# matthewdm0816/BridgeQA

Hardware: AMD Instinct MI355X
Metric: train samples/s (40k-pt scene + 512^2 view, bs16) (higher is better)
Workload: dtype bf16

## Files before the change

bridgeqa_amd/_ext.py:

```python
import ctypes
import os

import torch

from . import _cabi

_LIB_PATH = os.environ.get("BQHIP_LIB") or os.path.join(os.path.dirname(os.path.abspath(__file__)), "lib", "libbqhip.so")

if not os.path.exists(_LIB_PATH):
    raise ImportError(
        "bridgeqa_amd: %s is missing -- build it with `python -m bridgeqa_amd.build` "
        "(hipcc --offload-arch=gfx950). There is no CPU fallback." % _LIB_PATH)

_lib = ctypes.CDLL(_LIB_PATH)
_D = _cabi.DEFINES
_cabi.bind(_lib, ("bq_abi_version", "bq_last_error"))
ABI_VERSION = _D["BQHIP_ABI_VERSION"]
if _lib.bq_abi_version() != ABI_VERSION:
    raise ImportError("bridgeqa_amd: libbqhip.so ABI %d != %d (stale library: python -m bridgeqa_amd.build --force)"
                      % (_lib.bq_abi_version(), ABI_VERSION))
_cabi.bind(_lib)
_cabi.bind(_lib, _cabi.ADDITIVE_PROTOS)

DET_ROUTES = {
# ... 1092 lines not shown

GEMM_P_XC, GEMM_Q_XC, GEMM_OUT_F32, GEMM_BACKGROUND = (_D["BQ_GEMM_" + n] for n in ("P_XC", "Q_XC", "OUT_F32", "BACKGROUND"))
EPI_NONE, EPI_BIAS, EPI_BIAS_GELU, EPI_DGELU, EPI_BIAS_CE, EPI_ADD = (
    _D["BQ_GEMM_EPI_" + n] for n in ("NONE", "BIAS", "BIAS_GELU", "DGELU", "BIAS_CE", "ADD"))
GEMM_DET = _D["BQ_GEMM_DET"]
_GemmDesc = _cabi.STRUCTS["bq_gemm_desc"]
GEMM_TILE_ROWS = 1024


def _mat(t, name):
    if not t.is_cuda:
        raise RuntimeError("%s: CPU not supported (bridgeqa_amd has no CPU path)" % name)
    if t.dim() != 2 or t.stride(1) != 1:
        raise RuntimeError("%s must be a 2-D tensor with a contiguous last dimension" % name)
    return t


def _mat_rows(t, name):
    if not t.is_cuda:
        raise RuntimeError("%s: CPU not supported (bridgeqa_amd has no CPU path)" % name)
    if t.dim() == 2:
        if t.stride(1) != 1:
            raise RuntimeError("%s must have a contiguous last dimension" % name)
        return (t.shape[0], t.shape[1]), t.stride(0), 0, 0
    if t.dim() != 3 or t.stride(2) != 1:
        raise RuntimeError("%s must be (rows, cols) or a (batch, rows, cols) view with a contiguous last dimension" % name)
    B, R, C = t.shape
    ld, bs = t.stride(1), t.stride(0)
    if B == 1 or bs == R * ld:
        return (B * R, C), ld, 0, 0
    if bs < R * ld or bs % 8 or R > 65535:
        raise RuntimeError("%s: unsupported batched-row view (stride %s, shape %s)" % (name, t.stride(), tuple(t.shape)))
    return (B * R, C), ld, R, bs


TILE256_MIN_K = [2304]


def pick_tile(Ni, Nj, q_xc, mid_ok=False):
    if Nj >= GEMM_TILE_ROWS and Ni >= 256:
        return 128 if mid_ok else 256
    if q_xc or Nj > 512:
        return 64
    return 32


def gemm_grouped(problems, flags, epilogue=EPI_NONE, tile=None, fixed_order=False):
    if _det() or fixed_order:
        return _gemm_grouped_det(problems, flags, epilogue, tile)
    return _gemm_grouped_launch(problems, flags, epilogue, tile)


def _gemm_grouped_launch(problems, flags, epilogue, tile):
    pxc, qxc, f32 = bool(flags & GEMM_P_XC), bool(flags & GEMM_Q_XC), bool(flags & GEMM_OUT_F32)
    n = len(problems)
    arr = (_GemmDesc * n)()
    t_auto = 32
    any_map = False
    for k, pr in enumerate(problems):
        P, Q, out = _mat(pr["P"], "P"), pr["Q"], pr["out"]
        qshape, ldq, q_rpb, q_bs = _mat_rows(Q, "Q")
        oshape, ldo, o_rpb, o_bs = _mat_rows(out, "out")
        any_map = any_map or bool(q_rpb or o_rpb)
        if P.dtype != torch.bfloat16 or Q.dtype != torch.bfloat16:
            raise RuntimeError("gemm: operands must be bf16")
        if out.dtype != (torch.float32 if f32 else torch.bfloat16):
            raise RuntimeError("gemm: out must be %s" % ("float32" if f32 else "bfloat16"))
        Ni, Kc = (P.shape[1], P.shape[0]) if pxc else (P.shape[0], P.shape[1])
        Nj, Kq = (qshape[1], qshape[0]) if qxc else (qshape[0], qshape[1])
        Ni = int(pr.get("Ni", Ni))
        if (Kq != Kc and "Kc" not in pr) or tuple(oshape) != (Nj, Ni):
            raise RuntimeError("gemm: shape mismatch P%s Q%s out%s" % (tuple(P.shape), tuple(Q.shape), tuple(out.shape)))
        d = arr[k]
        d.P, d.Q, d.out = P.data_ptr(), Q.data_ptr(), out.data_ptr()
        bias, out2, aux, colsum = pr.get("bias"), pr.get("out2"), pr.get("aux"), pr.get("colsum")
        if bias is not None and (bias.dtype not in (torch.float32, torch.bfloat16) or bias.numel() != Ni
                                 or not bias.is_contiguous()):
            raise RuntimeError("gemm: bias must be a contiguous fp32 or bf16 (Ni,) tensor")
        d.bias_bf16 = int(bias is not None and bias.dtype == torch.bfloat16)
        n_cs = Nj if (pxc and qxc and f32) else Ni
        if epilogue != EPI_BIAS_CE and colsum is not None and (colsum.dtype != torch.float32 or colsum.numel() != n_cs
                                                               or not colsum.is_contiguous()):
            raise RuntimeError("gemm: colsum must be a contiguous fp32 (%d,) tensor" % n_cs)
        for t, nm in ((out2, "out2"), (aux, "aux")):
            if epilogue != EPI_BIAS_CE and t is not None and (t.dtype != torch.bfloat16 or t.shape != out.shape
                                                              or t.stride() != out.stride()):
                raise RuntimeError("gemm: %s must be bf16 and laid out like out" % nm)
        d.bias, d.out2, d.aux, d.colsum = _p(bias), _p(out2), _p(aux), _p(colsum)
        d.ldp, d.ldq, d.ldo = P.stride(0), ldq, ldo
        d.q_rpb, d.q_bstride, d.o_rpb, d.o_bstride = q_rpb, q_bs, o_rpb, o_bs
        d.accum = int(bool(pr.get("accum", False)))
        d.Ni, d.Nj, d.Kc = Ni, Nj, Kc
        d.p_bytes, d.q_bytes, d.ksplit = int(pr.get("p_bytes", 0)), int(pr.get("q_bytes", 0)), int(pr.get("ksplit", 1))
        if "Kc" in pr:
            d.Kc = int(pr["Kc"])
        mid_ok = (not qxc and not f32 and d.Kc >= 128 and colsum is None
                  and epilogue in (EPI_NONE, EPI_BIAS, EPI_BIAS_GELU, EPI_DGELU, EPI_ADD))
        all_mid_ok = mid_ok if k == 0 else (all_mid_ok and mid_ok)
        t_auto = max(t_auto, pick_tile(Ni, Nj, qxc, True))
    if t_auto == 128 and not all_mid_ok:
        t_auto = 256
    if (t_auto == 128 and TILE256_MIN_K[0] and not pxc and epilogue in (EPI_NONE, EPI_BIAS)
            and all(int(arr[k].Kc) >= TILE256_MIN_K[0] for k in range(n))):
        t_auto = 256
    if t_auto == 256 and any_map and tile is None and not (pxc and qxc and f32):
        t_auto = 64
    dev = problems[0]["out"].device
    if (tile or t_auto) != 128:
        flags &= ~GEMM_BACKGROUND
    with torch.cuda.device(dev):
        if (tile or t_auto) == 128 and n == 1 and (STREAMK[0] or STREAMK256[0]):
            _streamk_workspace(dev)
        _check(_lib.bq_gemm_bf16(arr, n, int(flags), int(epilogue), int(tile or t_auto), _stream()), "gemm_bf16")


def _gemm_grouped_det(problems, flags, epilogue, tile):
    if _det() and (STREAMK[0] or STREAMK256[0]):
        raise RuntimeError("gemm: stream-K is on (streamk_enable / streamk256_enable) while the deterministic mode is on")
    f32 = bool(flags & GEMM_OUT_F32)
    probs, folds, sums = [], [], []
    for pr in problems:
        ks = int(pr.get("ksplit", 1))
        if epilogue != EPI_BIAS_CE and ks > 1:
            out = pr["out"]
            if not f32 or pr.get("colsum") is not None or pr.get("accum") or out.dim() != 2 or out.stride(1) != 1:
                raise RuntimeError("gemm: a cut contraction in the deterministic mode needs fp32 plain-row out, no colsum or accum")
            slab = torch.empty(ks, out.shape[0], out.stride(0), dtype=torch.float32, device=out.device)
            folds.append((slab, out, ks))
            pr = dict(pr, out=slab[0, :, :out.shape[1]])
        elif not f32 and epilogue != EPI_BIAS_CE and pr.get("colsum") is not None:
            sums.append((pr["out"], pr["colsum"]))
            pr = dict(pr, colsum=None)
        probs.append(pr)
    _gemm_grouped_launch(probs, flags | GEMM_DET, epilogue, tile)
    for slab, out, ks in folds:
        R, C = out.shape
        with torch.cuda.device(out.device):
            _check(_det_entry("gemm_splitk_fold")(_p(slab), _p(out), None, ks, R, C, out.stride(0), _stream()),
                   "gemm_splitk_fold_det")
    if sums:
        _colsum_grouped_into([o.reshape(-1, o.shape[-1]) if o.dim() == 3 else o for o, _ in sums], [c for _, c in sums],
                             "gemm_epilogue_colsum")


STREAMK = [False]
STREAMK256 = [os.environ.get("BQ_GEMM_STREAMK256", "0") == "1"]
_SK_WS = {}


def _streamk_apply():
    on = STREAMK[0] or STREAMK256[0]
    _lib.bq_gemm_streamk_mode((1 if STREAMK[0] else 0) | (2 if STREAMK256[0] else 0))
    for (d, sp), (ws, st) in _SK_WS.items():
        with torch.cuda.device(d):
            _check(_lib.bq_gemm_set_workspace(_p(ws) if on else None, ws.numel() if on else 0, sp), "gemm_set_workspace")


def streamk_enable(flag):
    STREAMK[0] = bool(flag)
    _streamk_apply()


def streamk256_enable(flag):
    STREAMK256[0] = bool(flag)
    _streamk_apply()


_streamk_apply()


# ... 465 lines not shown
```

bridgeqa_amd/csrc/gemm.hip:

```cpp
#include "gemm_common.h"

namespace bq {

typedef unsigned u32x4_sk __attribute__((ext_vector_type(4)));

template <bool P_XC, bool Q_XC, int EPI, bool OUT_F32, bool SK = false>
__global__ __launch_bounds__(512) void gemm256_kernel(const GemmArgs args) {
  static_assert(!SK || (!P_XC && !Q_XC && !OUT_F32 && (EPI == EPI_NONE || EPI == EPI_BIAS)), "stream-K: K-contiguous operands, bf16 out");
  __shared__ __attribute__((aligned(16))) unsigned char smem[131072];
  __shared__ unsigned s_skflag;
  constexpr bool GTAB = !OUT_F32 && (EPI == EPI_BIAS_GELU || EPI == EPI_DGELU);
  __shared__ float s_gtab[GTAB ? GELU_TAB_N : 1];
  const int tid = threadIdx.x;
  const int lane = tid & 63;
  const int wave = __builtin_amdgcn_readfirstlane(tid >> 6);
  const int wr = wave >> 2, wc = wave & 3;

  const int nwg = args.total_tiles;
  auto xcd_order = [](int b, int n) {
    const int q = n >> 3, r = n & 7, x = b & 7;
    return (x < r ? x * (q + 1) : r * (q + 1) + (x - r) * q) + (b >> 3);
  };
  const int G = (int)gridDim.x;
  const int nkt_full = SK ? (args.p[0].Kc + 63) >> 6 : 1;
  const int U = SK ? nwg * nkt_full : 0;
  auto bound = [&](int x) {
    int b = (int)((long)x * U / G);
    const int r = b % nkt_full;
    return r == 1 ? b - 1 : (r == nkt_full - 1 ? b + 1 : b);
  };
  const int slot = SK ? xcd_order((int)blockIdx.x, G) : 0;
  int su = SK ? bound(slot) : 0;
  const int sue = SK ? bound(slot + 1) : 0;
  if (SK && su >= sue) return;
  for (;;) {
  int t, kb = 0, kseg = 0;
  if (SK) {
    t = su / nkt_full;
    kb = su - t * nkt_full;
    kseg = min(nkt_full - kb, sue - su);
  } else {
    t = xcd_order((int)blockIdx.x, nwg);
  }
  int pi = 0;
  for (int k = 1; k < args.n; ++k)
    if (t >= args.p[k].tile0) pi = k;
  const GemmProblem &pr = args.p[pi];
  const int tl = t - pr.tile0;
  const int tiles_j = (pr.Nj + 255) >> 8;
  const int bj = tiles_j - 1 - tl / pr.tiles_i(), bi = tl % pr.tiles_i();
  const int i0 = bi * 256, j0 = bj * 256;
  const int Ni = pr.Ni, Nj = pr.Nj, Kc = pr.Kc;
  const int ldp = pr.ldp, ldq = pr.ldq;
  const int nkt = SK ? kseg : (Kc + 63) >> 6;

  const auto rsP = __builtin_amdgcn_make_buffer_rsrc((void *)pr.P, 0, pr.p_bytes, 0x00020000);
  const auto rsQ = __builtin_amdgcn_make_buffer_rsrc((void *)pr.Q, 0, pr.q_bytes, 0x00020000);
  const int ur = wave * 8 + (lane >> 3);
  const int cp = lane & 7;
  unsigned voff[8];
#pragma unroll
  for (int u = 0; u < 4; ++u) {
    const int g = u & 1, half = u >> 1;
    if (!P_XC) {
      const int c = cp ^ (ur & 7);
      voff[u] = (unsigned)(((i0 + g * 128 + half * 64 + ur) * ldp + c * 8) * 2);
    } else {
      const int c = cp ^ (xg(ur) << 1);
      voff[u] = (unsigned)((ur * ldp + i0 + g * 128 + half * 64 + c * 8) * 2);
    }
  }
#pragma unroll
  for (int u = 0; u < 4; ++u) {
    const int h = u & 1, half = u >> 1;
    if (!Q_XC) {
      const int c = cp ^ (ur & 7);
      voff[4 + u] = (unsigned)(((j0 + h * 128 + (ur >> 5) * 64 + half * 32 + (ur & 31)) * ldq + c * 8) * 2);
    } else {
      const int c = cp ^ (xg(ur) << 1);
      voff[4 + u] = (unsigned)((ur * ldq + j0 + h * 128 + (c >> 2) * 64 + half * 32 + (c & 3) * 8) * 2);
    }
  }
  const unsigned p_step = P_XC ? (unsigned)(64 * ldp * 2) : 128u;
  const unsigned q_step = Q_XC ? (unsigned)(64 * ldq * 2) : 128u;
  if (SK) {
#pragma unroll
    for (int u = 0; u < 4; ++u) { voff[u] += (unsigned)kb * p_step; voff[4 + u] += (unsigned)kb * q_step; }
  }
  const unsigned lds_w = (unsigned)(wave * 1024);
  const int q_rpb = Q_XC ? (int)pr.q_rpb() : 0;
  const unsigned q_gap = (unsigned)((pr.q_bstride - q_rpb * ldq) * 2);
  int q_rl[2] = {ur, ur};

  auto stage_pair = [&](int u, int kt) {
    const bool live = kt < nkt;
    const unsigned base = (unsigned)((kt & 1) * 65536 + u * 8192) + lds_w;
#pragma unroll
    for (int d = 0; d < 2; ++d) {
      const unsigned vo = live ? voff[u + d] : 0x80000000u;
      __builtin_amdgcn_raw_ptr_buffer_load_lds(u < 4 ? rsP : rsQ, (lds_void_t *)(smem + base + d * 8192), 16, vo, 0, 0, 0);
      voff[u + d] += (u < 4) ? p_step : q_step;
    }
    if (Q_XC && u >= 4 && q_rpb != 0) {
      int &rl = q_rl[(u - 4) >> 1];
      rl += 64;
      const bool wrap = rl >= q_rpb;
      rl -= wrap ? q_rpb : 0;
      voff[u] += wrap ? q_gap : 0u;
      voff[u + 1] += wrap ? q_gap : 0u;
    }
  };

  const int row16 = lane & 15, q4 = lane >> 4;
  const int kc_base = row16 * 128 + ((q4 ^ (row16 & 7)) << 4);
  int xc_base[4];
  {
    const int q = (lane & 15) >> 2, p = lane & 3, g = (q >> 1) | ((q4 & 1) << 1);
#pragma unroll
    for (int s = 0; s < 4; ++s) xc_base[s] = (8 * q4 + q) * 128 + ((s ^ g) << 5) + 8 * p;
  }
  const int uA0 = wr * 8192, uA1 = (2 + wr) * 8192, uB0 = (4 + (wc >> 1)) * 8192, uB1 = (6 + (wc >> 1)) * 8192;
  const int bsub = (wc & 1) * 2;

  const int iw = i0 + wr * 128, jw = j0 + wc * 64;
  const bool vA0 = iw < Ni, vA1 = iw + 64 < Ni, vB0 = jw < Nj, vB1 = jw + 32 < Nj;

  f32x4 acc[8][4];
#pragma unroll
  for (int a = 0; a < 8; ++a)
#pragma unroll
    for (int b = 0; b < 4; ++b) acc[a][b] = f32x4{0.f, 0.f, 0.f, 0.f};

  constexpr bool QSUM = P_XC && Q_XC && OUT_F32;
  const bool do_qsum = QSUM && pr.colsum != nullptr && bi == 0 && wr == 0;
  f32x4 qs[4];
  bf16x8 ones;
#pragma unroll
  for (int b = 0; b < 4; ++b) qs[b] = f32x4{0.f, 0.f, 0.f, 0.f};
#pragma unroll
  for (int e = 0; e < 8; ++e) ones[e] = (__bf16)1.0f;
#define BQ_MFMA_QSUM(FB, BO)                                                                          \
  if (QSUM && do_qsum) {                                                                              \
    _Pragma("unroll") for (int kk = 0; kk < 2; ++kk) _Pragma("unroll") for (int b = 0; b < 2; ++b)    \
        qs[BO + b] = __builtin_amdgcn_mfma_f32_16x16x32_bf16(ones, FB[b][kk], qs[BO + b], 0, 0, 0);   \
  }

  stage_pair(0, 0); stage_pair(4, 0); stage_pair(6, 0); stage_pair(2, 0); stage_pair(0, 1); stage_pair(4, 1); stage_pair(6, 1);
  if (GTAB) gelu_tab_fill<EPI == EPI_DGELU>(s_gtab, tid, 512);
  asm volatile("s_waitcnt vmcnt(8)" ::: "memory");
  BQ_BARRIER();
  if (wr == 1) BQ_BARRIER();

  bf16x8 fa[4][2], fb0[2][2], fb1[2][2];
  const unsigned smem_lds = lds_addr_of(smem);
#define BQ_MFMA_Q(AO, FB, BO)                                                                         \
  _Pragma("unroll") for (int kk = 0; kk < 2; ++kk) _Pragma("unroll") for (int a = 0; a < 4; ++a)      \
      _Pragma("unroll") for (int b = 0; b < 2; ++b) acc[AO + a][BO + b] =                             \
          __builtin_amdgcn_mfma_f32_16x16x32_bf16(fa[a][kk], FB[b][kk], acc[AO + a][BO + b], 0, 0, 0);
#define BQ_PHASE_SYNC_A()                                   \
  asm volatile("s_waitcnt vmcnt(8)" ::: "memory");          \
  asm volatile("s_waitcnt lgkmcnt(0)" ::: "memory");        \
  BQ_BARRIER();                                             \
  __builtin_amdgcn_sched_barrier(0);                        \
  __builtin_amdgcn_s_setprio(1);
#define BQ_PHASE_SYNC_B()                                   \
  __builtin_amdgcn_s_setprio(0);                            \
  BQ_BARRIER();

  for (int kt = 0; kt < nkt; ++kt) {
    const unsigned buf = smem_lds + (unsigned)((kt & 1) * 65536);
    if (vA0) {
#pragma unroll
      for (int a = 0; a < 4; ++a)
#pragma unroll
        for (int kk = 0; kk < 2; ++kk) fa[a][kk] = read_frag_asm<P_XC>(buf + uA0, a, kk, kc_base, xc_base);
    }
    if (vB0) {
#pragma unroll
      for (int b = 0; b < 2; ++b)
#pragma unroll
        for (int kk = 0; kk < 2; ++kk) fb0[b][kk] = read_frag_asm<Q_XC>(buf + uB0, bsub + b, kk, kc_base, xc_base);
    }
    if (vB1) {
#pragma unroll
      for (int b = 0; b < 2; ++b)
#pragma unroll
        for (int kk = 0; kk < 2; ++kk) fb1[b][kk] = read_frag_asm<Q_XC>(buf + uB1, bsub + b, kk, kc_base, xc_base);
    }
    stage_pair(2, kt + 1);
    BQ_PHASE_SYNC_A();
    if (vA0 && vB0) { BQ_MFMA_Q(0, fb0, 0) }
    if (vB0) { BQ_MFMA_QSUM(fb0, 0) }
    if (vA0 && vB1) { BQ_MFMA_Q(0, fb1, 2) }
    if (vB1) { BQ_MFMA_QSUM(fb1, 2) }
    BQ_PHASE_SYNC_B();
    if (vA1) {
#pragma unroll
      for (int a = 0; a < 4; ++a)
#pragma unroll
        for (int kk = 0; kk < 2; ++kk) fa[a][kk] = read_frag_asm<P_XC>(buf + uA1, a, kk, kc_base, xc_base);
    }
    stage_pair(0, kt + 2); stage_pair(4, kt + 2); stage_pair(6, kt + 2);
    BQ_PHASE_SYNC_A();
    if (vA1 && vB1) { BQ_MFMA_Q(4, fb1, 2) }
    if (vA1 && vB0) { BQ_MFMA_Q(4, fb0, 0) }
    BQ_PHASE_SYNC_B();
  }
  if (wr == 0) BQ_BARRIER();
  asm volatile("s_waitcnt vmcnt(0)" ::: "memory");
  BQ_BARRIER();

  if (SK && kseg != nkt_full) {
    unsigned *tick = (unsigned *)args.sk_ws + 2 * t;
    const int t0 = t * nkt_full, t1 = t0 + nkt_full;
    int s_lo = slot, s_hi = slot;
    while (s_lo > 0 && bound(s_lo) > t0) --s_lo;
    while (s_hi + 1 < G && bound(s_hi + 1) < t1) ++s_hi;
    const int n_part = s_hi - s_lo + 1;
    if (tid == 0) s_skflag = __hip_atomic_fetch_add(tick, 1u, __ATOMIC_RELAXED, __HIP_MEMORY_SCOPE_AGENT);
    __syncthreads();
    const unsigned arrived = (unsigned)__builtin_amdgcn_readfirstlane((int)s_skflag);
    constexpr unsigned SLAB256 = 256u * 256u * 4u;
    const auto rsW = __builtin_amdgcn_make_buffer_rsrc((char *)args.sk_ws + SK_TICKET_BYTES, 0, 0x7fffffffu, 0x00020000);
    auto slab_off = [&](int sl) { return (unsigned)(2 * sl + (bound(sl) >= t0 ? 0 : 1)) * SLAB256; };
    if (arrived != (unsigned)(n_part - 1)) {
      const unsigned base = slab_off(slot) + (unsigned)(tid * 16);
#pragma unroll
      for (int a = 0; a < 8; ++a)
#pragma unroll
        for (int b = 0; b < 4; ++b)
          __builtin_amdgcn_raw_buffer_store_b128(__builtin_bit_cast(u32x4_sk, acc[a][b]), rsW, base + (unsigned)((a * 4 + b) * 8192), 0, 16);
      asm volatile("s_waitcnt vmcnt(0)" ::: "memory");
      __syncthreads();
      if (tid == 0) __hip_atomic_fetch_add(tick + 1, 1u, __ATOMIC_RELAXED, __HIP_MEMORY_SCOPE_AGENT);
      su += kseg;
      if (su >= sue) return;
      continue;
    }
    if (tid == 0) {
      for (int spin = 0; spin < (1 << 22) && __hip_atomic_load(tick + 1, __ATOMIC_RELAXED, __HIP_MEMORY_SCOPE_AGENT) != (unsigned)(n_part - 1); ++spin)
        __builtin_amdgcn_s_sleep(4);
      __hip_atomic_store(tick, 0u, __ATOMIC_RELAXED, __HIP_MEMORY_SCOPE_AGENT);
      __hip_atomic_store(tick + 1, 0u, __ATOMIC_RELAXED, __HIP_MEMORY_SCOPE_AGENT);
    }
    __syncthreads();
    for (int sl = s_lo; sl <= s_hi; ++sl) {
      if (sl == slot) continue;
      const unsigned base = slab_off(sl) + (unsigned)(tid * 16);
#pragma unroll
      for (int a0 = 0; a0 < 8; a0 += 2) {
        u32x4_sk part[8];
#pragma unroll
        for (int e = 0; e < 8; ++e) part[e] = __builtin_amdgcn_raw_buffer_load_b128(rsW, base + (unsigned)((a0 * 4 + e) * 8192), 0, 16);
        asm volatile("s_waitcnt vmcnt(0)" ::: "memory");
        __builtin_amdgcn_sched_barrier(0);
#pragma unroll
        for (int e = 0; e < 8; ++e) acc[a0 + (e >> 2)][e & 3] += __builtin_bit_cast(f32x4, part[e]);
      }
    }
  }

  const int ldo = pr.ldo;
  if (OUT_F32) {
    float *out = reinterpret_cast<float *>(pr.out);
    if (QSUM && do_qsum && q4 == 0) {
#pragma unroll
      for (int b = 0; b < 4; ++b) {
        const int j = jw + b * 16 + row16;
        if (j < Nj) pr.colsum[j] = qs[b][0];
      }
    }
#pragma unroll
    for (int b = 0; b < 4; ++b) {
      const int j = jw + b * 16 + row16;
#pragma unroll
      for (int a = 0; a < 8; ++a) {
        const int i = iw + a * 16 + q4 * 4;
        if (j < Nj && i < Ni) {
          float4 *dst = reinterpret_cast<float4 *>(out + (long)j * ldo + i);
          const f32x4 v = acc[a][b];
          *dst = make_float4(v[0], v[1], v[2], v[3]);
        }
      }
    }
    return;
  }
  if (EPI == EPI_BIAS_CE) {
    const int n_valid = pr.ksplit();
    float *part = reinterpret_cast<float *>(pr.out2) + (long)(bi * 2 + wr) * Nj * 3;
    const int *tgt = reinterpret_cast<const int *>(pr.aux);
#pragma unroll
    for (int b = 0; b < 4; ++b) {
      const int j = jw + b * 16 + row16;
      const int t = j < Nj ? tgt[j] : -100;
      float m = -INFINITY, sz = 0.f;
#pragma unroll
      for (int a = 0; a < 8; ++a) {
        const int i = iw + a * 16 + q4 * 4;
        float bv[4] = {0.f, 0.f, 0.f, 0.f};
        if (pr.bias != nullptr && i < Ni) load_bias4(pr, i, bv);
#pragma unroll
        for (int r = 0; r < 4; ++r) {
          const float z = acc[a][b][r] + bv[r];
          if (i + r < n_valid) {
            m = fmaxf(m, z);
            sz += z;
            if (i + r == t) pr.colsum[j] = z;
          }
        }
      }
      float se = 0.f;
#pragma unroll
      for (int a = 0; a < 8; ++a) {
        const int i = iw + a * 16 + q4 * 4;
        float bv[4] = {0.f, 0.f, 0.f, 0.f};
        if (pr.bias != nullptr && i < Ni) load_bias4(pr, i, bv);
#pragma unroll
        for (int r = 0; r < 4; ++r)
          if (i + r < n_valid) se += __builtin_amdgcn_exp2f((acc[a][b][r] + bv[r] - m) * 1.4426950408889634f);
      }
#pragma unroll
      for (int sh = 16; sh <= 32; sh <<= 1) {
        const float mo = __shfl_xor(m, sh), so = __shfl_xor(se, sh), zo = __shfl_xor(sz, sh);
        const float mn = fmaxf(m, mo);
        const float fa = m == -INFINITY ? 0.f : __builtin_amdgcn_exp2f((m - mn) * 1.4426950408889634f);
        const float fb = mo == -INFINITY ? 0.f : __builtin_amdgcn_exp2f((mo - mn) * 1.4426950408889634f);
        se = se * fa + so * fb;
        m = mn;
        sz += zo;
      }
      if (q4 == 0 && j < Nj) {
        part[(long)j * 3 + 0] = m;
        part[(long)j * 3 + 1] = se;
        part[(long)j * 3 + 2] = sz;
      }
    }
  }
  unsigned char *ep = smem + wave * 16384;
  __bf16 *outb = reinterpret_cast<__bf16 *>(pr.out);
  const int npass = (EPI == EPI_BIAS_GELU) ? 2 : 1;
  const bool want_colsum = EPI != EPI_BIAS_CE && pr.colsum != nullptr;
#pragma unroll 1
  for (int pass = 0; pass < npass; ++pass) {
    if (EPI == EPI_DGELU || EPI == EPI_ADD) {
      float cs[8][4];
#pragma unroll
      for (int a = 0; a < 8; ++a)
#pragma unroll
        for (int r = 0; r < 4; ++r) cs[a][r] = 0.f;
      const auto rsX = __builtin_amdgcn_make_buffer_rsrc((void *)pr.aux, 0, (int)((long)Nj * ldo * 2), 0x00020000);
      uint2 yy[2][8];
      auto fetch = [&](int b, uint2(&dst)[8]) {
        const unsigned off = (unsigned)(((jw + b * 16 + row16) * ldo + iw + q4 * 4) * 2);
// ... 749 lines not shown
        }
        if (long_k) {
          hipLaunchKernelGGL((gemm64_kernel<32, P_XC, Q_XC, EPI, OUT_F32, 2>), dim3(ga.total_tiles), dim3(256), 0, st, ga);
          return 0;
        }
      }
      hipLaunchKernelGGL((gemm64_kernel<32, P_XC, Q_XC, EPI, OUT_F32>), dim3(ga.total_tiles), dim3(256), 0, st, ga);
    } else {
      return -1;
    }
  }
  return 0;
}

template <bool P_XC, bool Q_XC, int EPI>
static int launch_det_variant(const GemmArgs &ga, int tile, hipStream_t st) {
  if (tile == 64) {
    hipLaunchKernelGGL((gemm64_kernel_det<64, P_XC, Q_XC, EPI>), dim3(ga.total_tiles), dim3(256), 0, st, ga);
    return 0;
  }
  if constexpr (!Q_XC) {
    hipLaunchKernelGGL((gemm64_kernel_det<32, P_XC, Q_XC, EPI>), dim3(ga.total_tiles), dim3(256), 0, st, ga);
    return 0;
  }
  return -1;
}

static int launch_gemm(const GemmArgs &ga, int flags, int epi, int tile, hipStream_t st) {
  const bool pxc = flags & BQ_GEMM_P_XC, qxc = flags & BQ_GEMM_Q_XC, f32 = flags & BQ_GEMM_OUT_F32;
  if ((flags & BQ_GEMM_DET) && f32 && tile != 256 && tile != 128) {
    if (!pxc && !qxc && epi == EPI_NONE) return launch_det_variant<false, false, EPI_NONE>(ga, tile, st);
    if (!pxc && !qxc && epi == EPI_BIAS) return launch_det_variant<false, false, EPI_BIAS>(ga, tile, st);
    if (pxc && !qxc && epi == EPI_NONE) return launch_det_variant<true, false, EPI_NONE>(ga, tile, st);
    if (pxc && qxc && epi == EPI_NONE) return launch_det_variant<true, true, EPI_NONE>(ga, tile, st);
    return -1;
  }
  constexpr int long_k_tiles = 12;
  bool long_k = long_k_tiles > 0 && tile != 256 && ga.total_tiles <= 2048;
  for (int k = 0; k < ga.n; ++k) long_k = long_k && ga.p[k].Kc >= 64 * long_k_tiles;
  if (tile == 128 && (gemm_sk_mode() & 2) && !(flags & (BQ_GEMM_BACKGROUND | BQ_GEMM_DET)) && ga.n == 1 && !pxc && !qxc && !f32 &&
      (epi == EPI_NONE || epi == EPI_BIAS) && ga.p[0].colsum == nullptr && ga.p[0].q_rpb() == 0 && ga.p[0].o_rpb() == 0) {
    const GemmProblem &p0 = ga.p[0];
    const int cus = device_cus();
    const int nkt = (p0.Kc + 63) >> 6, tiles = ((p0.Ni + 255) / 256) * ((p0.Nj + 255) / 256);
    const long units = (long)tiles * nkt;
    const int rounds = (tiles + cus - 1) / cus;
    long ws_bytes = 0;
    void *ws = gemm_sk_workspace(st, &ws_bytes);
    if (ws != nullptr && nkt >= 24 && tiles >= cus / 2 && units / cus >= 16 && (long)rounds * nkt * cus >= units * 115 / 100 &&
        8L * tiles <= SK_TICKET_BYTES && ws_bytes >= SK_TICKET_BYTES + 2L * cus * 256 * 256 * 4) {
      GemmArgs g2 = ga;
      g2.sk_ws = ws;
      g2.total_tiles = tiles;
      g2.p[0].tile0 = 0;
      g2.p[0].tiles_ks = (p0.Ni + 255) / 256;
      if (epi == EPI_NONE) hipLaunchKernelGGL((gemm256_kernel<false, false, EPI_NONE, false, true>), dim3(cus), dim3(512), 0, st, g2);
      else hipLaunchKernelGGL((gemm256_kernel<false, false, EPI_BIAS, false, true>), dim3(cus), dim3(512), 0, st, g2);
      return 0;
    }
  }
  if (tile == 128)
    return launch_gemm_mid(ga, pxc, qxc, f32, epi, (flags & BQ_GEMM_BACKGROUND) != 0, st);
  if (!pxc && !qxc && !f32) {
    if (epi == EPI_NONE) return launch_variant<false, false, EPI_NONE, false>(ga, tile, st, long_k);
    if (epi == EPI_BIAS) return launch_variant<false, false, EPI_BIAS, false>(ga, tile, st, long_k);
    if (epi == EPI_BIAS_GELU) return launch_variant<false, false, EPI_BIAS_GELU, false>(ga, tile, st, long_k);
    if (epi == EPI_DGELU) return launch_variant<false, false, EPI_DGELU, false>(ga, tile, st, long_k);
    if (epi == EPI_ADD) return launch_variant<false, false, EPI_ADD, false>(ga, tile, st, long_k);
    if (epi == EPI_BIAS_CE && tile == 256) {
      hipLaunchKernelGGL((gemm256_kernel<false, false, EPI_BIAS_CE, false>), dim3(ga.total_tiles), dim3(512), 0, st, ga);
      return 0;
    }
  } else if (!pxc && !qxc && f32) {
    if (epi == EPI_NONE && tile != 256) return launch_variant<false, false, EPI_NONE, true>(ga, tile, st);
    if (epi == EPI_BIAS && tile != 256) return launch_variant<false, false, EPI_BIAS, true>(ga, tile, st);
  } else if (pxc && !qxc && f32) {
    if (epi == EPI_NONE && tile != 256) return launch_variant<true, false, EPI_NONE, true>(ga, tile, st);
  } else if (pxc && !qxc && !f32) {
    if (epi == EPI_NONE) return launch_variant<true, false, EPI_NONE, false>(ga, tile, st, long_k);
    if (epi == EPI_DGELU) return launch_variant<true, false, EPI_DGELU, false>(ga, tile, st, long_k);
    if (epi == EPI_ADD) return launch_variant<true, false, EPI_ADD, false>(ga, tile, st, long_k);
  } else if (pxc && qxc && f32) {
    if (epi == EPI_NONE) return launch_variant<true, true, EPI_NONE, true>(ga, tile, st);
  }
  return -1;
}

}

extern "C" int bq_gemm_max_problems(void) { return bq::GEMM_MAX_PROBLEMS; }

extern "C" int bq_gemm_bf16(const bq_gemm_desc *d, int n, int flags, int epilogue, int tile, void *stream) {
  using namespace bq;
  BQ_REQUIRE(d != nullptr && n >= 1, BQ_EINVAL, "bq_gemm_bf16: no problems");
  BQ_REQUIRE(tile == 256 || tile == 128 || tile == 64 || tile == 32, BQ_EINVAL,
             "bq_gemm_bf16: tile must be 256, 128 (= 256 x 128), 64 or 32 (got %d)", tile);
  const bool pxc = flags & BQ_GEMM_P_XC, qxc = flags & BQ_GEMM_Q_XC, f32 = flags & BQ_GEMM_OUT_F32;
  BQ_REQUIRE(!(flags & BQ_GEMM_BACKGROUND) || tile == 128, BQ_EINVAL, "bq_gemm_bf16: BQ_GEMM_BACKGROUND needs tile 128");
  const bool det = flags & BQ_GEMM_DET;
  BQ_REQUIRE(!det || tile != 128 || gemm_sk_mode() == 0, BQ_EINVAL,
             "bq_gemm_bf16: BQ_GEMM_DET with a stream-K mode on (bq_gemm_streamk_mode)");
  hipStream_t st = (hipStream_t)stream;
  int done = 0;
  while (done < n) {
    GemmArgs ga;
    ga.n = 0;
    ga.total_tiles = 0;
    while (done < n && ga.n < GEMM_MAX_PROBLEMS) {
      const bq_gemm_desc &s = d[done];
      BQ_REQUIRE(s.P && s.Q && s.out, BQ_EINVAL, "bq_gemm_bf16: null operand (problem %d)", done);
      BQ_REQUIRE(s.Ni > 0 && s.Nj > 0 && s.Kc > 0, BQ_EINVAL, "bq_gemm_bf16: empty problem %d", done);
      BQ_REQUIRE(s.ldp % 8 == 0 && s.ldq % 8 == 0, BQ_EINVAL, "bq_gemm_bf16: operand leading dimensions must be multiples of 8 elements");
      BQ_REQUIRE(s.Ni % 8 == 0 && s.ldo % (f32 ? 4 : 8) == 0, BQ_EINVAL, "bq_gemm_bf16: Ni and ldo must be multiples of 8 (Ni = %d, ldo = %d)", s.Ni, s.ldo);
      BQ_REQUIRE(!qxc || s.Nj % 8 == 0, BQ_EINVAL, "bq_gemm_bf16: a contraction-major Q needs Nj %% 8 == 0 (Nj = %d)", s.Nj);
      BQ_REQUIRE((pxc && qxc) || s.Kc % 64 == 0, BQ_EINVAL,
                 "bq_gemm_bf16: a K-contiguous operand needs Kc %% 64 == 0 (Kc = %d; zero-pad the other operand and pass "
                 "p_bytes / q_bytes when the rows are shorter)", s.Kc);
      BQ_REQUIRE(((uintptr_t)s.P % 16 == 0) && ((uintptr_t)s.Q % 16 == 0) && ((uintptr_t)s.out % 16 == 0), BQ_EINVAL,
                 "bq_gemm_bf16: operands must be 16-byte aligned");
      BQ_REQUIRE(epilogue != EPI_BIAS_GELU || s.out2, BQ_EINVAL, "bq_gemm_bf16: BIAS_GELU needs out2");
      BQ_REQUIRE(epilogue != EPI_DGELU || s.aux, BQ_EINVAL, "bq_gemm_bf16: DGELU needs aux");
      BQ_REQUIRE(epilogue != EPI_ADD || s.aux, BQ_EINVAL, "bq_gemm_bf16: ADD needs aux");
      BQ_REQUIRE((epilogue != EPI_ADD && epilogue != EPI_DGELU && tile != 128) || ((long)s.Nj + 256) * s.ldo * (f32 ? 4 : 2) < 0x7FFFFFFFL,
                 BQ_EINVAL, "bq_gemm_bf16: out / aux larger than 2 GB (problem %d)", done);
      const long pb = pxc ? ((long)(s.Kc - 1) * s.ldp + s.Ni) * 2 : ((long)(s.Ni - 1) * s.ldp + s.Kc) * 2;
      long qb = qxc ? ((long)(s.Kc - 1) * s.ldq + s.Nj) * 2 : ((long)(s.Nj - 1) * s.ldq + s.Kc) * 2;
      const int tj = tile == 256 ? 256 : tile, ti = (tile == 256 || tile == 128) ? 256 : 64;
      BQ_REQUIRE(s.q_rpb >= 0 && s.o_rpb >= 0 && s.q_rpb <= 65535 && s.o_rpb <= 65535, BQ_EINVAL,
                 "bq_gemm_bf16: q_rpb / o_rpb must be in 0..65535 (problem %d)", done);
      long q_span = 0, o_span = 0;
      if (s.q_rpb > 0) {
        const long rows = qxc ? s.Kc : s.Nj, cols = qxc ? s.Nj : s.Kc;
        BQ_REQUIRE(rows % s.q_rpb == 0 && s.q_bstride % 8 == 0 && (long)s.q_bstride >= (long)s.q_rpb * s.ldq, BQ_EINVAL,
                   "bq_gemm_bf16: q map: rows %ld must be whole batches of q_rpb = %d rows, q_bstride %% 8 == 0 and >= q_rpb * ldq",
                   rows, s.q_rpb);
        BQ_REQUIRE(tile != 256 || (qxc && s.q_rpb >= 64), BQ_EINVAL,
                   "bq_gemm_bf16: tile 256 maps only the contraction rows of a contraction-major Q, q_rpb >= 64");
        BQ_REQUIRE(tile != 128 || !qxc, BQ_EINVAL, "bq_gemm_bf16: tile 128 has no map on a contraction-major Q");
        q_span = (rows / s.q_rpb - 1) * (long)s.q_bstride + (long)(s.q_rpb - 1) * s.ldq + cols;
        qb = q_span * 2;
      }
      if (s.o_rpb > 0) {
        BQ_REQUIRE(s.Nj % s.o_rpb == 0 && s.o_bstride % 8 == 0 && (long)s.o_bstride >= (long)s.o_rpb * s.ldo, BQ_EINVAL,
                   "bq_gemm_bf16: o map: Nj = %d must be whole batches of o_rpb = %d rows, o_bstride %% 8 == 0 and >= o_rpb * ldo",
                   s.Nj, s.o_rpb);
        BQ_REQUIRE(tile != 256 && epilogue != EPI_BIAS_CE && s.colsum == nullptr, BQ_EINVAL,
                   "bq_gemm_bf16: an output map needs tile 128, 64 or 32 and no column sums");
        o_span = (long)(s.Nj / s.o_rpb) * s.o_bstride;
        BQ_REQUIRE((o_span + 256L * s.ldo) * (f32 ? 4 : 2) < 0x7FFFFFFFL, BQ_EINVAL, "bq_gemm_bf16: mapped out larger than 2 GB");
      }
      BQ_REQUIRE(!s.accum || (f32 && tile != 256 && tile != 128), BQ_EINVAL, "bq_gemm_bf16: accum needs fp32 out and tile 64 / 32");
      BQ_REQUIRE(pb + (long)ti * s.ldp * 2 < 0x7FFFFFFFL && qb + (long)tj * s.ldq * 2 + (s.q_rpb > 0 ? 2L * s.q_bstride * 2 : 0) < 0x7FFFFFFFL,
                 BQ_EINVAL, "bq_gemm_bf16: operand larger than 2 GB (problem %d)", done);
      BQ_REQUIRE(!det || f32 || epilogue == EPI_BIAS_CE || !s.colsum, BQ_EINVAL,
                 "bq_gemm_bf16: BQ_GEMM_DET: column sums of a bf16 output are float atomics (use bq_colsum_grouped_det_bf16)");
      BQ_REQUIRE(!det || epilogue == EPI_BIAS_CE || s.ksplit <= 1 || (!s.colsum && !s.accum && s.o_rpb == 0), BQ_EINVAL,
                 "bq_gemm_bf16: BQ_GEMM_DET: a cut contraction takes no colsum, accum or output map (problem %d)", done);
      GemmProblem &g = ga.p[ga.n];
      g.P = (const __bf16 *)s.P; g.Q = (const __bf16 *)s.Q; g.out = s.out; g.bias = s.bias; g.out2 = s.out2;
      g.aux = (const __bf16 *)s.aux; g.colsum = s.colsum;
      g.ldp = s.ldp; g.ldq = s.ldq; g.ldo = s.ldo; g.Ni = s.Ni; g.Nj = s.Nj; g.Kc = s.Kc;
      g.flags = (s.bias_bf16 != 0 ? 1 : 0) | (s.accum != 0 ? 2 : 0);
      g.rpb_pack = (int)((unsigned)s.q_rpb | ((unsigned)s.o_rpb << 16));
      g.q_bstride = s.q_bstride; g.o_bstride = s.o_bstride;
      g.p_bytes = (unsigned)(s.p_bytes > 0 ? s.p_bytes : pb);
      g.q_bytes = (unsigned)((s.q_bytes > 0 && s.q_rpb == 0) ? s.q_bytes : qb);
      int ks_ = 1;
      if (epilogue == EPI_BIAS_CE) {
        BQ_REQUIRE(s.out2 && s.aux && s.colsum && s.ksplit > 0 && s.ksplit <= s.Ni && s.ksplit <= 65535 && tile == 256, BQ_EINVAL,
                   "bq_gemm_bf16: the cross-entropy epilogue needs out2 (partials), aux (targets), colsum (target logits), "
                   "ksplit = valid vocabulary entries (<= 65535), tile 256");
        ks_ = s.ksplit;
      } else {
        BQ_REQUIRE(s.ksplit <= 1 || (f32 && tile != 256), BQ_EINVAL, "bq_gemm_bf16: ksplit needs fp32 out and tile 64");
        BQ_REQUIRE(s.ksplit <= 65535, BQ_ELIMIT, "bq_gemm_bf16: ksplit = %d > 65535", s.ksplit);
        BQ_REQUIRE(s.ksplit <= 1 || epilogue == EPI_NONE, BQ_EINVAL, "bq_gemm_bf16: ksplit needs the NONE epilogue");
        ks_ = (f32 && tile != 256 && s.ksplit > 1) ? s.ksplit : 1;
      }
      BQ_REQUIRE((s.Ni + ti - 1) / ti <= 65535, BQ_ELIMIT, "bq_gemm_bf16: Ni = %d too wide", s.Ni);
      g.tiles_ks = (int)((unsigned)((s.Ni + ti - 1) / ti) | ((unsigned)ks_ << 16));
      g.tile0 = ga.total_tiles;
      ga.total_tiles += g.tiles_i() * ((s.Nj + tj - 1) / tj) * (epilogue == EPI_BIAS_CE ? 1 : g.ksplit());
      ++ga.n;
      ++done;
    }
    BQ_REQUIRE(launch_gemm(ga, flags, epilogue, tile, st) == 0, BQ_EINVAL,
               "bq_gemm_bf16: unsupported combination flags=%d epilogue=%d tile=%d", flags, epilogue, tile);
    int rc = check_launch("gemm_bf16");
    if (rc) return rc;
  }
  return 0;
}

extern "C" int bq_colsum_grouped_bf16(const bq_colsum_desc *d, int n, void *stream) {
  using namespace bq;
  BQ_REQUIRE(d != nullptr && n >= 1, BQ_EINVAL, "bq_colsum_grouped_bf16: no problems");
  hipStream_t st = (hipStream_t)stream;
  int done = 0;
  while (done < n) {
    ColsumArgs ca;
    ca.n = 0;
    int wgs = 0;
    while (done < n && ca.n < COLSUM_MAX_PROBLEMS) {
      const bq_colsum_desc &s = d[done];
      BQ_REQUIRE(s.g && s.out && s.M > 0 && s.N > 0, BQ_EINVAL, "bq_colsum_grouped_bf16: bad problem %d", done);
      BQ_REQUIRE(s.N % 8 == 0 && s.ld % 8 == 0 && ((uintptr_t)s.g % 16 == 0), BQ_EINVAL,
                 "bq_colsum_grouped_bf16: N and ld must be multiples of 8, g 16-byte aligned");
      ColsumProblem &c = ca.p[ca.n];
      c.g = (const __bf16 *)s.g; c.out = s.out; c.M = s.M; c.N = s.N; c.ld = s.ld;
      c.cblocks = (s.N + 255) / 256;
      c.wg0 = wgs;
      wgs += c.cblocks * ((s.M + COLSUM_ROWS - 1) / COLSUM_ROWS);
      ++ca.n;
      ++done;
    }
    hipLaunchKernelGGL(colsum_grouped_kernel, dim3(wgs), dim3(256), 0, st, ca);
    int rc = check_launch("colsum_grouped");
    if (rc) return rc;
  }
  return 0;
}

static long colsum_det_wgs(const bq_colsum_desc *d, int n) {
  long wgs = 0;
  for (int k = 0; k < n; ++k) wgs += (long)((d[k].N + 255) / 256) * ((d[k].M + bq::COLSUM_ROWS - 1) / bq::COLSUM_ROWS);
  return wgs;
}
extern "C" long bq_colsum_grouped_det_floats(const bq_colsum_desc *d, int n) {
  return (d && n > 0) ? 256L * colsum_det_wgs(d, n) : 0;
}

extern "C" int bq_colsum_grouped_det_bf16(const bq_colsum_desc *d, int n, float *partial, void *stream) {
  using namespace bq;
  BQ_REQUIRE(d != nullptr && n >= 1, BQ_EINVAL, "bq_colsum_grouped_det_bf16: no problems");
  BQ_REQUIRE(partial != nullptr, BQ_EINVAL, "bq_colsum_grouped_det_bf16: no workspace");
// ... 357 lines not shown
```

bridgeqa_amd/fusion_wgrad.py:

```python
import os

import torch
import torch.nn.functional as F

from .fusion_state import *
from .fusion_state import __all__ as _state_all

_NATIVE_GEMM = [True]


def _rows(t):
    t2 = t.reshape(-1, t.shape[-1])
    if t2.dtype != torch.bfloat16:
        t2 = t2.to(torch.bfloat16)
    if t2.stride(1) != 1 or t2.stride(0) % 8 or t2.data_ptr() % 16:
        t2 = t2.contiguous()
    return t2


def _native_ok(t, N, K):
    return _NATIVE_GEMM[0] and t.is_cuda and compute_dtype() == torch.bfloat16 and K % 64 == 0 and N % 8 == 0


def _native_dx_ok(t, N, K):
    return _NATIVE_GEMM[0] and t.is_cuda and compute_dtype() == torch.bfloat16 and N % 64 == 0 and K % 8 == 0


def _f32_bias(bias):
    if bias is None:
        return None
    if bias.dtype == torch.float32 and bias.is_contiguous():
        return bias.detach()
    return _shadow(bias)


def _mm_f32(a, b):
    return torch.mm(a.float(), b.float()) if not a.is_cuda else torch.mm(a, b, out_dtype=torch.float32)


def _dw_db(g2, x2, need_dw, need_db):
    dw = db = None
    native = g2.is_cuda and g2.dtype == torch.bfloat16 and x2.dtype == torch.bfloat16 and g2.shape[1] % 8 == 0 \
        and x2.shape[1] % 8 == 0 and _NATIVE_GEMM[0]
    if need_dw:
        if native:
            from . import _ext
            dw = _ext.gemm_dw(_rows(g2), _rows(x2), tile=256 if g2.shape[0] >= _BIG_ROWS else 64)
        else:
            dw = _mm_f32(g2.t(), x2)
    if need_db:
        if native:
            from . import _ext
            db = _ext.colsum_grouped([_rows(g2)])[0]
        else:
            db = g2.sum(0, dtype=torch.float32)
    return dw, db


_DEFER = [None]
_BIG_ROWS = 1024


def begin_deferred_wgrad():
    _DEFER[0] = []


def _accumulate_grad(p, g):
    if p is None or not p.requires_grad:
        return
    if p.grad is None:
        p.grad = g
    else:
        p.grad.add_(g)


def take_deferred_wgrad():
    items, _DEFER[0] = _DEFER[0], None
    return items or []


def flush_deferred_wgrad():
    flush_deferred_items(take_deferred_wgrad())


_PLAN_CACHE = {}
_PLAN_WGRAD = [True]
_QSUM = [True]
_QSUM64 = [True]
_DW_TILE = [256]
_SHORT_DW_MIN_ROWS = [64]
_SHORT_DW_TILE = [256]


def plan_big_launches(tiles, cus, max_problems=36, moved_cost=0.011):
    key = (tuple(tiles), cus, max_problems)
    hit = _PLAN_CACHE.get(key)
    if hit is not None:
        return hit
    n = len(tiles)
    rounds = lambda t: -(-t // cus) if t > 0 else 0
    order = sorted(range(n), key=lambda k: tiles[k])
    default = [list(range(n))[i:i + max_problems] for i in range(0, n, max_problems)]
    best = (sum(rounds(sum(tiles[k] for k in g)) for g in default), default, [])
    if n <= 2 * max_problems:
        for m in range(0, min(6, n)):
            moved = order[:m]
            rest = order[m:]
            cost_moved = moved_cost * sum(tiles[k] for k in moved)
            by_size = {}
            for k in rest:
                by_size.setdefault(tiles[k], []).append(k)
            sizes = sorted(by_size)
            if len(sizes) > 5:
                break
            total, cnt = sum(tiles[k] for k in rest), len(rest)
            combos = [[]]
            for sz in sizes:
                combos = [c + [x] for c in combos for x in range(len(by_size[sz]) + 1)]
                if len(combos) > 50000:
                    combos = None
                    break
            if combos is None:
                break
            for c in combos:
                nb = sum(c)
                if nb > max_problems or cnt - nb > max_problems:
                    continue
                tb = sum(x * sz for x, sz in zip(c, sizes))
                cost = rounds(tb) + rounds(total - tb) + cost_moved
                if cost < best[0] - 1e-9:
                    gb = [k for x, sz in zip(c, sizes) for k in by_size[sz][:x]]
                    ga = [k for x, sz in zip(c, sizes) for k in by_size[sz][x:]]
                    best = (cost, [g for g in (ga, gb) if g], list(moved))
    plan = (best[1], best[2])
    _PLAN_CACHE[key] = plan
    return plan


def _nrows(t):
    return t.shape[0] if t.dim() == 2 else t.shape[0] * t.shape[1]


def flush_deferred_items(items):
    if not items:
        return
    from . import _ext
    flags = _ext.GEMM_P_XC | _ext.GEMM_Q_XC | _ext.GEMM_OUT_F32
    items = [tuple(it) + (None,) * (5 - len(it)) for it in items]
    dws = [None] * len(items)
    prim = [k for k, it in enumerate(items) if it[4] is None]
    second = [k for k, it in enumerate(items) if it[4] is not None]
    big = [k for k in prim if _nrows(items[k][0]) >= _BIG_ROWS]
    small = [k for k in prim if _nrows(items[k][0]) < _BIG_ROWS]
    if _PLAN_WGRAD[0]:
        big.sort(key=lambda k: -_nrows(items[k][0]))
    groups = [big] if big else []
    if big and _PLAN_WGRAD[0]:
        tj = _DW_TILE[0]
        tiles = [-(-items[k][0].shape[-1] // tj) * -(-items[k][1].shape[-1] // 256) for k in big]
        cus = torch.cuda.get_device_properties(items[big[0]][0].device).multi_processor_count
        plan_groups, moved = plan_big_launches(tiles, cus * (256 // tj))
        groups = [[big[j] for j in g] for g in plan_groups]
        small = small + [big[j] for j in moved]
    dbs = {}
    mid = []
    if _SHORT_DW_TILE[0] in (128, 256):
        min_rows = max(_SHORT_DW_MIN_ROWS[0], 128 if _SHORT_DW_TILE[0] == 128 else 1)
        ok = lambda it: (min_rows <= _nrows(it[0]) < _BIG_ROWS and it[0].dim() == 2 and it[0].shape[-1] >= 128
                         and it[1].shape[-1] >= 256)
        mid = [k for k in small if ok(items[k])]
        small = [k for k in small if not ok(items[k])]
    for tile, idx_groups in ((_DW_TILE[0], groups), (_SHORT_DW_TILE[0], [mid] if mid else []), (64, [small] if small else [])):
        for idx in idx_groups:
            probs = []
            for k in idx:
                g2, x2 = items[k][0], items[k][1]
                dws[k] = torch.empty(g2.shape[-1], x2.shape[-1], dtype=torch.float32, device=g2.device)
                pr = dict(P=x2, Q=g2, out=dws[k])
                if items[k][3] is not None and _QSUM[0] and (tile != 64 or _QSUM64[0]):
                    dbs[k] = torch.empty(g2.shape[-1], dtype=torch.float32, device=g2.device)
                    pr["colsum"] = dbs[k]
                probs.append(pr)
            _ext.gemm_grouped(probs, flags, _ext.EPI_NONE, tile)
    with_b = [k for k in prim if items[k][3] is not None and k not in dbs]
    if with_b:
        dbs.update(zip(with_b, _ext.colsum_grouped([items[k][0].reshape(-1, items[k][0].shape[-1]) for k in with_b])))
    if second:
        probs = []
        for k in second:
            g2, x2, pk = items[k][0], items[k][1], items[k][4]
            pr = dict(P=x2, Q=g2, out=dws[pk], accum=True)
            if items[pk][3] is not None:
                pr["colsum"] = dbs[pk]
            probs.append(pr)
        _ext.gemm_grouped(probs, flags, _ext.EPI_NONE, 64)
    for k in prim:
        g2, x2, ws, bs = items[k][:4]
        n = g2.shape[-1] // len(ws)
        for j, w in enumerate(ws):
            _accumulate_grad(w, dws[k][j * n:(j + 1) * n] if len(ws) > 1 else dws[k].view(w.shape))
            if bs is not None:
                _accumulate_grad(bs[j], dbs[k][j * n:(j + 1) * n] if len(ws) > 1 else dbs[k])


def _defer_ok(g2, x2):
    return (_DEFER[0] is not None and _NATIVE_GEMM[0] and g2.is_cuda and g2.dtype == torch.bfloat16
            and x2.dtype == torch.bfloat16 and g2.shape[1] % 8 == 0 and x2.shape[1] % 8 == 0)


def _park(g2, x2, ws, bs):
    _DEFER[0].append((_rows(g2), _rows(x2), ws, bs))


def _park_two(g_a, x_a, g_b, x_b, ws, bs):
    d = _DEFER[0]
    d.append((g_a, _rows(x_a), ws, bs))
    d.append((g_b, _rows(x_b), ws, bs, len(d) - 1))



__all__ = [n for n in list(globals()) if not n.startswith("__")]
```

Baseline: 503.9.

## Add fp32 add-epilogue to tile-256 weight-gradient GEMM for second accumulation pass

Adds an EPI_ADD variant of the 256-tile weight-gradient kernel with fp32 output. It reads the existing fp32 partial gradient as aux, adds the new product in the epilogue and accumulates column sums. The q-row map also accepts batch sizes below 64 rows by wrapping multiple batches per step. The second-pass wgrad GEMMs that qualify now use this big-tile kernel instead of the 64-tile accumulate path, aiming for better MFMA efficiency on those problems. The cost is an extra fp32 read of the output, in-place read-modify-write aliasing, and integer divisions in the staging loop.

```diff
diff --git a/bridgeqa_amd/_ext.py b/bridgeqa_amd/_ext.py
--- a/bridgeqa_amd/_ext.py
+++ b/bridgeqa_amd/_ext.py
@@ -1198,10 +1198,12 @@
         if epilogue != EPI_BIAS_CE and colsum is not None and (colsum.dtype != torch.float32 or colsum.numel() != n_cs
                                                                or not colsum.is_contiguous()):
             raise RuntimeError("gemm: colsum must be a contiguous fp32 (%d,) tensor" % n_cs)
+        add32 = f32 and epilogue == EPI_ADD
         for t, nm in ((out2, "out2"), (aux, "aux")):
-            if epilogue != EPI_BIAS_CE and t is not None and (t.dtype != torch.bfloat16 or t.shape != out.shape
+            want = torch.float32 if (add32 and nm == "aux") else torch.bfloat16
+            if epilogue != EPI_BIAS_CE and t is not None and (t.dtype != want or t.shape != out.shape
                                                               or t.stride() != out.stride()):
-                raise RuntimeError("gemm: %s must be bf16 and laid out like out" % nm)
+                raise RuntimeError("gemm: %s must be %s and laid out like out" % (nm, "fp32" if want == torch.float32 else "bf16"))
         d.bias, d.out2, d.aux, d.colsum = _p(bias), _p(out2), _p(aux), _p(colsum)
         d.ldp, d.ldq, d.ldo = P.stride(0), ldq, ldo
         d.q_rpb, d.q_bstride, d.o_rpb, d.o_bstride = q_rpb, q_bs, o_rpb, o_bs
diff --git a/bridgeqa_amd/csrc/gemm.hip b/bridgeqa_amd/csrc/gemm.hip
--- a/bridgeqa_amd/csrc/gemm.hip
+++ b/bridgeqa_amd/csrc/gemm.hip
@@ -7,6 +7,8 @@
 template <bool P_XC, bool Q_XC, int EPI, bool OUT_F32, bool SK = false>
 __global__ __launch_bounds__(512) void gemm256_kernel(const GemmArgs args) {
   static_assert(!SK || (!P_XC && !Q_XC && !OUT_F32 && (EPI == EPI_NONE || EPI == EPI_BIAS)), "stream-K: K-contiguous operands, bf16 out");
+  constexpr bool ADD32 = OUT_F32 && EPI == EPI_ADD;
+  static_assert(!ADD32 || (P_XC && Q_XC), "the fp32 add epilogue belongs to the weight-gradient form");
   __shared__ __attribute__((aligned(16))) unsigned char smem[131072];
   __shared__ unsigned s_skflag;
   constexpr bool GTAB = !OUT_F32 && (EPI == EPI_BIAS_GELU || EPI == EPI_DGELU);
@@ -78,7 +80,10 @@
       voff[4 + u] = (unsigned)(((j0 + h * 128 + (ur >> 5) * 64 + half * 32 + (ur & 31)) * ldq + c * 8) * 2);
     } else {
       const int c = cp ^ (xg(ur) << 1);
-      voff[4 + u] = (unsigned)((ur * ldq + j0 + h * 128 + (c >> 2) * 64 + half * 32 + (c & 3) * 8) * 2);
+      if (ADD32)
+        voff[4 + u] = (mapped_row(ur, ldq, (int)pr.q_rpb(), pr.q_bstride) + (unsigned)(j0 + h * 128 + (c >> 2) * 64 + half * 32 + (c & 3) * 8)) * 2u;
+      else
+        voff[4 + u] = (unsigned)((ur * ldq + j0 + h * 128 + (c >> 2) * 64 + half * 32 + (c & 3) * 8) * 2);
     }
   }
   const unsigned p_step = P_XC ? (unsigned)(64 * ldp * 2) : 128u;
@@ -91,6 +96,7 @@
   const int q_rpb = Q_XC ? (int)pr.q_rpb() : 0;
   const unsigned q_gap = (unsigned)((pr.q_bstride - q_rpb * ldq) * 2);
   int q_rl[2] = {ur, ur};
+  if (ADD32 && q_rpb != 0) q_rl[0] = q_rl[1] = ur % q_rpb;
 
   auto stage_pair = [&](int u, int kt) {
     const bool live = kt < nkt;
@@ -104,10 +110,17 @@
     if (Q_XC && u >= 4 && q_rpb != 0) {
       int &rl = q_rl[(u - 4) >> 1];
       rl += 64;
-      const bool wrap = rl >= q_rpb;
-      rl -= wrap ? q_rpb : 0;
-      voff[u] += wrap ? q_gap : 0u;
-      voff[u + 1] += wrap ? q_gap : 0u;
+      if (ADD32) {
+        const int nb = rl / q_rpb;
+        rl -= nb * q_rpb;
+        voff[u] += (unsigned)nb * q_gap;
+        voff[u + 1] += (unsigned)nb * q_gap;
+      } else {
+        const bool wrap = rl >= q_rpb;
+        rl -= wrap ? q_rpb : 0;
+        voff[u] += wrap ? q_gap : 0u;
+        voff[u + 1] += wrap ? q_gap : 0u;
+      }
     }
   };
 
@@ -267,8 +280,36 @@
 #pragma unroll
       for (int b = 0; b < 4; ++b) {
         const int j = jw + b * 16 + row16;
-        if (j < Nj) pr.colsum[j] = qs[b][0];
-      }
+        if (ADD32) {
+          if (j < Nj) pr.colsum[j] = pr.aux != nullptr ? pr.colsum[j] + qs[b][0] : qs[b][0];
+        } else {
+          if (j < Nj) pr.colsum[j] = qs[b][0];
+        }
+      }
+    }
+    if (ADD32 && pr.aux != nullptr) {
+      const float *add = reinterpret_cast<const float *>(pr.aux);
+#pragma unroll
+      for (int b = 0; b < 4; ++b) {
+        const int j = jw + b * 16 + row16;
+        float4 base[8];
+#pragma unroll
+        for (int a = 0; a < 8; ++a) {
+          const int i = iw + a * 16 + q4 * 4;
+          base[a] = make_float4(0.f, 0.f, 0.f, 0.f);
+          if (j < Nj && i < Ni) base[a] = *reinterpret_cast<const float4 *>(add + (long)j * ldo + i);
+        }
+#pragma unroll
+        for (int a = 0; a < 8; ++a) {
+          const int i = iw + a * 16 + q4 * 4;
+          if (j < Nj && i < Ni) {
+            const f32x4 v = acc[a][b];
+            *reinterpret_cast<float4 *>(out + (long)j * ldo + i) =
+                make_float4(base[a].x + v[0], base[a].y + v[1], base[a].z + v[2], base[a].w + v[3]);
+          }
+        }
+      }
+      return;
     }
 #pragma unroll
     for (int b = 0; b < 4; ++b) {
@@ -1184,6 +1225,10 @@
     if (epi == EPI_ADD) return launch_variant<true, false, EPI_ADD, false>(ga, tile, st, long_k);
   } else if (pxc && qxc && f32) {
     if (epi == EPI_NONE) return launch_variant<true, true, EPI_NONE, true>(ga, tile, st);
+    if (epi == EPI_ADD && tile == 256) {
+      hipLaunchKernelGGL((gemm256_kernel<true, true, EPI_ADD, true>), dim3(ga.total_tiles), dim3(512), 0, st, ga);
+      return 0;
+    }
   }
   return -1;
 }
@@ -1222,7 +1267,10 @@
                  "bq_gemm_bf16: operands must be 16-byte aligned");
       BQ_REQUIRE(epilogue != EPI_BIAS_GELU || s.out2, BQ_EINVAL, "bq_gemm_bf16: BIAS_GELU needs out2");
       BQ_REQUIRE(epilogue != EPI_DGELU || s.aux, BQ_EINVAL, "bq_gemm_bf16: DGELU needs aux");
-      BQ_REQUIRE(epilogue != EPI_ADD || s.aux, BQ_EINVAL, "bq_gemm_bf16: ADD needs aux");
+      BQ_REQUIRE(epilogue != EPI_ADD || s.aux || f32, BQ_EINVAL, "bq_gemm_bf16: ADD needs aux");
+      BQ_REQUIRE(epilogue != EPI_ADD || !f32 || (pxc && qxc && tile == 256), BQ_EINVAL,
+                 "bq_gemm_bf16: ADD with fp32 out is the weight-gradient form (P_XC | Q_XC) on tile 256");
+      BQ_REQUIRE(epilogue != EPI_ADD || !f32 || (uintptr_t)s.aux % 16 == 0, BQ_EINVAL, "bq_gemm_bf16: aux must be 16-byte aligned");
       BQ_REQUIRE((epilogue != EPI_ADD && epilogue != EPI_DGELU && tile != 128) || ((long)s.Nj + 256) * s.ldo * (f32 ? 4 : 2) < 0x7FFFFFFFL,
                  BQ_EINVAL, "bq_gemm_bf16: out / aux larger than 2 GB (problem %d)", done);
       const long pb = pxc ? ((long)(s.Kc - 1) * s.ldp + s.Ni) * 2 : ((long)(s.Ni - 1) * s.ldp + s.Kc) * 2;
@@ -1236,8 +1284,9 @@
         BQ_REQUIRE(rows % s.q_rpb == 0 && s.q_bstride % 8 == 0 && (long)s.q_bstride >= (long)s.q_rpb * s.ldq, BQ_EINVAL,
                    "bq_gemm_bf16: q map: rows %ld must be whole batches of q_rpb = %d rows, q_bstride %% 8 == 0 and >= q_rpb * ldq",
                    rows, s.q_rpb);
-        BQ_REQUIRE(tile != 256 || (qxc && s.q_rpb >= 64), BQ_EINVAL,
-                   "bq_gemm_bf16: tile 256 maps only the contraction rows of a contraction-major Q, q_rpb >= 64");
+        BQ_REQUIRE(tile != 256 || (qxc && (s.q_rpb >= 64 || (f32 && epilogue == EPI_ADD))), BQ_EINVAL,
+                   "bq_gemm_bf16: tile 256 maps only the contraction rows of a contraction-major Q, q_rpb >= 64 (any q_rpb with "
+                   "the fp32 ADD epilogue)");
         BQ_REQUIRE(tile != 128 || !qxc, BQ_EINVAL, "bq_gemm_bf16: tile 128 has no map on a contraction-major Q");
         q_span = (rows / s.q_rpb - 1) * (long)s.q_bstride + (long)(s.q_rpb - 1) * s.ldq + cols;
         qb = q_span * 2;
@@ -1252,7 +1301,7 @@
         BQ_REQUIRE((o_span + 256L * s.ldo) * (f32 ? 4 : 2) < 0x7FFFFFFFL, BQ_EINVAL, "bq_gemm_bf16: mapped out larger than 2 GB");
       }
       BQ_REQUIRE(!s.accum || (f32 && tile != 256 && tile != 128), BQ_EINVAL, "bq_gemm_bf16: accum needs fp32 out and tile 64 / 32");
-      BQ_REQUIRE(pb + (long)ti * s.ldp * 2 < 0x7FFFFFFFL && qb + (long)tj * s.ldq * 2 + (s.q_rpb > 0 ? 2L * s.q_bstride * 2 : 0) < 0x7FFFFFFFL,
+      BQ_REQUIRE(pb + (long)ti * s.ldp * 2 < 0x7FFFFFFFL && qb + (long)tj * s.ldq * 2 + (s.q_rpb > 0 ? (2L + (s.q_rpb < 64 ? 64 / s.q_rpb : 0)) * s.q_bstride * 2 : 0) < 0x7FFFFFFFL,
                  BQ_EINVAL, "bq_gemm_bf16: operand larger than 2 GB (problem %d)", done);
       BQ_REQUIRE(!det || f32 || epilogue == EPI_BIAS_CE || !s.colsum, BQ_EINVAL,
                  "bq_gemm_bf16: BQ_GEMM_DET: column sums of a bf16 output are float atomics (use bq_colsum_grouped_det_bf16)");
diff --git a/bridgeqa_amd/fusion_wgrad.py b/bridgeqa_amd/fusion_wgrad.py
--- a/bridgeqa_amd/fusion_wgrad.py
+++ b/bridgeqa_amd/fusion_wgrad.py
@@ -90,6 +90,9 @@
 _DW_TILE = [256]
 _SHORT_DW_MIN_ROWS = [64]
 _SHORT_DW_TILE = [256]
+
+
+_SECOND_DW_ADD256 = [True]
 
 
 def plan_big_launches(tiles, cus, max_problems=36, moved_cost=0.011):
@@ -186,14 +189,24 @@
     if with_b:
         dbs.update(zip(with_b, _ext.colsum_grouped([items[k][0].reshape(-1, items[k][0].shape[-1]) for k in with_b])))
     if second:
-        probs = []
-        for k in second:
-            g2, x2, pk = items[k][0], items[k][1], items[k][4]
-            pr = dict(P=x2, Q=g2, out=dws[pk], accum=True)
-            if items[pk][3] is not None:
-                pr["colsum"] = dbs[pk]
-            probs.append(pr)
-        _ext.gemm_grouped(probs, flags, _ext.EPI_NONE, 64)
+        add256 = []
+        if _SECOND_DW_ADD256[0] and _SHORT_DW_TILE[0] == 256:
+            add256 = [k for k in second if _nrows(items[k][0]) >= _SHORT_DW_MIN_ROWS[0] and items[k][0].shape[-1] >= 128
+                      and items[k][1].shape[-1] >= 256 and items[k][0].shape[-1] % 8 == 0]
+        for tile, idx in ((256, add256), (64, [k for k in second if k not in add256])):
+            probs = []
+            for k in idx:
+                g2, x2, pk = items[k][0], items[k][1], items[k][4]
+                pr = dict(P=x2, Q=g2, out=dws[pk])
+                if tile == 256:
+                    pr["aux"] = dws[pk]
+                else:
+                    pr["accum"] = True
+                if items[pk][3] is not None:
+                    pr["colsum"] = dbs[pk]
+                probs.append(pr)
+            if probs:
+                _ext.gemm_grouped(probs, flags, _ext.EPI_ADD if tile == 256 else _ext.EPI_NONE, tile)
     for k in prim:
         g2, x2, ws, bs = items[k][:4]
         n = g2.shape[-1] // len(ws)
```

New measurement: 508.2 (median of 6 runs). About the same (+0.9%).
